# Rinoahu/SwiftOrtho

Measured on AMD Instinct MI355X. Metric: M query-aa/s scanned all-vs-all, higher is better.
Workload: dtype u8/int16/int32 (5-bit packed residues, packed 16-bit score-only DP, int32 traced DP); 1 GPU; BASELINE config 3: 100000 synthetic proteins x 300 aa self-search, seed 11111011111, aa9, -M 120000000, -c 50000 (2 chunks), -e 1e-5, -v 500; query_aa=30007201, rows=1618760

## Files before the change

### swiftortho_amd/csrc/k_ixsort.hip

```cpp
#include "common.h"
#include "kernels.h"

#define IXS_G 512
#define IXS_T1 1024
#define IXS_BINS_MAX 8192
#define IXS_W 16384
#define IXS_T2 512

static inline int ixs_wsh(u32 NC) {
    int wsh = 0;
    while ((((u64)NC + (1ull << wsh) - 1) >> wsh) > IXS_BINS_MAX) ++wsh;
    return wsh;
}
u32 ixsort_bins(u32 NC) { return (u32)(((u64)NC + (1ull << ixs_wsh(NC)) - 1) >> ixs_wsh(NC)); }
size_t ixsort_plan_elems(u32 NC) { return (size_t)ixsort_bins(NC) * IXS_G + 1; }

__device__ __forceinline__ u32 ixs_col() { return (blockIdx.x & 7u) * (IXS_G / 8) + (blockIdx.x >> 3); }
__device__ __forceinline__ void ixs_slice(u32 E, u32& lo, u32& hi) {
    const u64 per = (((u64)E + IXS_G - 1) / IXS_G + 3) & ~3ull;
    lo = (u32)min((u64)E, per * ixs_col()), hi = (u32)min((u64)E, per * (ixs_col() + 1));
}

__global__ __launch_bounds__(IXS_T1) void k_ixs_count(const u32* __restrict__ keys, u32 E, int wsh, u32 nbins, u32* __restrict__ plan ) {
    __shared__ u32 s_cnt[IXS_BINS_MAX];
    for (u32 i = threadIdx.x; i < nbins; i += IXS_T1) s_cnt[i] = 0;
    __syncthreads();
    u32 lo, hi;
    ixs_slice(E, lo, hi);
    for (u32 i = lo + threadIdx.x; i < hi; i += IXS_T1) {
        const u32 k = keys[i];
        if (k != 0xFFFFFFFFu) atomicAdd(&s_cnt[k >> wsh], 1u);
    }
    __syncthreads();
    for (u32 i = threadIdx.x; i < nbins; i += IXS_T1) plan[(size_t)i * IXS_G + ixs_col()] = s_cnt[i];
    if (blockIdx.x == 0 && threadIdx.x == 0) plan[(size_t)nbins * IXS_G] = 0;
}

__global__ __launch_bounds__(IXS_T1) void k_ixs_scatter(const u32* __restrict__ keys, const u64* __restrict__ vals, u32 E, int wsh, u32 nbins,
                                                       const u32* __restrict__ plan , u32* __restrict__ tk, u64* __restrict__ tv) {
    __shared__ u32 s_cur[IXS_BINS_MAX];
    for (u32 i = threadIdx.x; i < nbins; i += IXS_T1) s_cur[i] = plan[(size_t)i * IXS_G + ixs_col()];
    __syncthreads();
    u32 lo, hi;
    ixs_slice(E, lo, hi);
    for (u32 i = lo + threadIdx.x; i < hi; i += IXS_T1) {
        const u32 k = keys[i];
        if (k == 0xFFFFFFFFu) continue;
        const u32 at = atomicAdd(&s_cur[k >> wsh], 1u);
        tk[at] = k, tv[at] = vals[i];
    }
}

__device__ __forceinline__ void ixs_group(const u32* sk, const u64* sv, u32 a, u32 b, u32 idbase, u32* __restrict__ dk,
                                          u64* __restrict__ dv, u32* s_cnt, u32* s_ws) {
    const int tid = threadIdx.x, lane = tid & 63, w = tid >> 6;
    constexpr int PER = IXS_W / IXS_T2;
    for (int i = tid; i < IXS_W; i += IXS_T2) s_cnt[i] = 0;
    __syncthreads();
    for (u32 i = a + (u32)tid; i < b; i += IXS_T2) atomicAdd(&s_cnt[sk[i] - idbase], 1u);
    __syncthreads();
    {
        u32 c[PER], tot = 0;
#pragma unroll
        for (int k = 0; k < PER; ++k) c[k] = s_cnt[tid * PER + k], tot += c[k];
        u32 inc = tot;
#pragma unroll
        for (int o = 1; o < 64; o <<= 1) {
            const u32 x = __shfl_up(inc, o);
            if (lane >= o) inc += x;
        }
        if (lane == 63) s_ws[w] = inc;
        __syncthreads();
        u32 run = a + inc - tot;
        for (int k = 0; k < w; ++k) run += s_ws[k];
#pragma unroll
        for (int k = 0; k < PER; ++k) {
            s_cnt[tid * PER + k] = run;
            run += c[k];
        }
    }
    __syncthreads();
    for (u32 i = a + (u32)tid; i < b; i += IXS_T2) {
        const u32 k = sk[i];
        const u32 at = atomicAdd(&s_cnt[k - idbase], 1u);
        dk[at] = k, dv[at] = sv[i];
    }
    __syncthreads();
}

__global__ __launch_bounds__(IXS_T2) void k_ixs_bin(const u32* __restrict__ tk, const u64* __restrict__ tv, const u32* __restrict__ plan, int wsh,
                                                    u32* ak, u64* av ,
                                                    u32* __restrict__ ok, u64* __restrict__ ov) {
    __shared__ u32 s_cnt[IXS_W];
    __shared__ u32 s_ws[IXS_T2 / 64];
    __shared__ u32 s_sub[34];
    const u32 bin = blockIdx.x;
    const u32 a = plan[(size_t)bin * IXS_G], b = plan[(size_t)(bin + 1) * IXS_G];
    if (a == b) return;
    const u32 idbase = bin << wsh;
    if (wsh <= 14) {
        ixs_group(tk, tv, a, b, idbase, ok, ov, s_cnt, s_ws);
        return;
    }
    const u32 nsub = 1u << (wsh - 14);
    const int tid = threadIdx.x;
    if (tid < 34) s_sub[tid] = 0;
    __syncthreads();
    for (u32 i = a + (u32)tid; i < b; i += IXS_T2) atomicAdd(&s_sub[(tk[i] - idbase) >> 14], 1u);
    __syncthreads();
    if (tid == 0) {
        u32 run = a;
        for (u32 j = 0; j <= nsub; ++j) {
            const u32 c = j < nsub ? s_sub[j] : 0u;
            s_sub[j] = run;
            run += c;
        }
    }
    __syncthreads();
    u32 sub_lo[32];
    for (u32 j = 0; j < nsub; ++j) sub_lo[j] = s_sub[j];
    const u32 sub_end = s_sub[nsub];
    __syncthreads();
    for (u32 i = a + (u32)tid; i < b; i += IXS_T2) {
        const u32 k = tk[i];
        const u32 at = atomicAdd(&s_sub[(k - idbase) >> 14], 1u);
        ak[at] = k, av[at] = tv[i];
    }
    __threadfence();
    __syncthreads();
    for (u32 j = 0; j < nsub; ++j) {
        const u32 sa = sub_lo[j], sb = j + 1 < nsub ? sub_lo[j + 1] : sub_end;
        if (sa < sb) ixs_group(ak, av, sa, sb, idbase + (j << 14), ok, ov, s_cnt, s_ws);
    }
}

const u32* ixsort_count(const u32* kin, u32 n, u32 NC, u32* plan, u32* scan_tmp, hipStream_t st) {
    const int wsh = ixs_wsh(NC);
    const u32 nbins = ixsort_bins(NC);
    hipLaunchKernelGGL(k_ixs_count, dim3(IXS_G), dim3(IXS_T1), 0, st, kin, n, wsh, nbins, plan);
    scan_u32(plan, plan, (size_t)nbins * IXS_G + 1, false, scan_tmp, st);
    return plan + (size_t)nbins * IXS_G;
}
void ixsort_finish(u32* kin, u64* vin, u32 n, u32 NC, const u32* plan, u32* tk, u64* tv, u32* kout, u64* vout, hipStream_t st) {
    if (!n) return;
    const int wsh = ixs_wsh(NC);
    const u32 nbins = ixsort_bins(NC);
    hipLaunchKernelGGL(k_ixs_scatter, dim3(IXS_G), dim3(IXS_T1), 0, st, kin, vin, n, wsh, nbins, plan, tk, tv);
    hipLaunchKernelGGL(k_ixs_bin, dim3(nbins), dim3(IXS_T2), 0, st, tk, tv, plan, wsh, kin, vin, kout, vout);
}
void ixsort_pairs(u32* kin, u64* vin, u32 E, u32 NC, u32* plan, u32* scan_tmp, u32* tk, u64* tv, u32* kout, u64* vout, hipStream_t st) {
    if (!E) return;
    (void)ixsort_count(kin, E, NC, plan, scan_tmp, st);
    ixsort_finish(kin, vin, E, NC, plan, tk, tv, kout, vout, st);
}
```

### swiftortho_amd/csrc/tune.h

```cpp
#pragma once
#include <cstdlib>

#define SOHIT_TUNE_TABLE(X)                                                                                                                                     \
                                                                                                                              \
    X(B, ug1, "SOHIT_UG1", 1, "bucketed passes: singleton groups to k_ungap1 (0: everything to k_ungap)")                                                     \
    X(B, ug1_chain, "SOHIT_UG1_CHAIN", 1, "... and the groups of two and more hits to k_ungap2 (0: to k_ungap, which then skips the singletons)")              \
    X(B, count_steps, "SOHIT_UG_COUNT", 0, "counting instances of the extension kernels: so_counters.ungap_steps, groups_single, groups_chain")                \
    X(B, ungapq, "SOHIT_UNGAPQ", 1, "sparse passes of queries up to 512 residues: hits alone on their diagonal by k_ungapq, a wave per query (0: every hit through the sorted keys)")     \
    X(I, uq_cache, "SOHIT_UQ_CACHE", -1, "... its hit ordinals per query whose index entries stay in registers between the two walks, in steps of 64 (-1: the compiled 1024; 0: every entry read twice; tests move the boundary)") \
    X(I, uq_chains, "SOHIT_UQ_CHAINS", -1, "... what it leaves over sorted per query (k_uqsort_wave: a wave's registers, k_uqsort_wg: a workgroup's LDS) and chained by k_ungap2 from the list of group heads (0: library segmented sort + k_ungap + k_first_touch; N > 0: the largest tier holds N keys -- tests reach the in-place instance with small inputs)") \
    X(B, ug_w32, "SOHIT_UG_W32", 1, "bucketed passes hand k_ungap the buckets' 32-bit words (0: 64-bit keys; no k_ungap1 then)")                               \
                                                                                                             \
    X(B, bucket, "SOHIT_BUCKET", 1, "bucketed diagonal binning (0: every pass on the sorted path)")                                                            \
    X(I, bucket_min, "SOHIT_BUCKET_MIN", 192, "hits per bucket below which a pass takes the sorted path (0: bucketed whenever possible)")                      \
    X(I, bucket_avg, "SOHIT_BUCKET_AVG", 2560, "average bucket size the band-range width is chosen for")                                                       \
    X(I, count_tab, "SOHIT_COUNT_TAB", 1, "bucketed passes: hits per (tile, range) from the range boundaries of the ordered index buckets when a batch brings a chunk two passes and more (0: always the counting pass over the entries; 2: always both, compared -- tests; 3: always)") \
    X(B, bucket_best, "SOHIT_BUCKET_BEST", 1, "best diagonal per subject by the per-bucket reduction (0: sort of the pass records)")                           \
    X(B, bands, "SOHIT_BANDS", 1, "diagonal bands follow the subjects' lengths (0: one band per subject)")                                                     \
    X(B, lk_wide, "SOHIT_LK_WIDE", 0, "8-byte index addends whatever the field widths")                                                                        \
    X(B, qclass, "SOHIT_QCLASS", 1, "queries of a batch in length-class order (0: file order)")                                                                \
    X(B, pass_merge, "SOHIT_PASS_MERGE", 1, "neighbouring length classes that take the sorted path anyway share one pass")                                     \
    X(B, ksc_lazy, "SOHIT_KSC_LAZY", 1, "k-mer orders computed for the queries that reach their frequency cap, when they do (a query below it keeps every window whatever the order; 0: for every query, with the batch)") \
    X(B, bounds_ahead, "SOHIT_BOUNDS_AHEAD", 1, "the next chunk's bucket bounds (k_bounds) on the side stream beside this chunk's seed stage (0: in front of its own)")     \
    X(I, segsort, "SOHIT_SEGSORT", 1, "sorted path: segmented sort of the keys inside each query (0: device-wide sort)")                                        \
    X(I, write_threads, "SOHIT_WRITE_THREADS", 48, "so_write_sc: formatter threads (at most the host's cores)")                                                                          \
                                                                                                                                 \
    X(I, cand_limit, "SOHIT_CAND_LIMIT", 0, "tests: candidate-store size at which a batch is split (0: 2^32 - 16)")                                            \
                                                                                                                                         \
    X(B, align_pk, "SOHIT_ALIGN_PK", 1, "packed 16-bit score-only aligner where the scores fit")                                                               \
    X(B, align_lane, "SOHIT_ALIGN_LANE", 1, "score-only rounds: one lane per alignment pair (k_align_lane) when no sequence reaches 4096 residues (0: k_align_pk)")            \
    X(I, align_lane_min, "SOHIT_ALIGN_LANE_MIN", 1 << 18, "... for rounds of at least this many packed tasks (below: k_align_pk; tests: 0)")                 \
    X(B, align_sort, "SOHIT_ALIGN_SORT", 1, "launch lists ordered by band rows")                                                                               \
    X(I, trace_wave_rows, "SOHIT_TRACE_WAVE_ROWS", 1024, "traceback: bands of this many rows and more are walked by a wave of their own (0: never)")         \
    X(I, trace_wave_max, "SOHIT_TRACE_WAVE_MAX", 32768, "... among the first this many positions of a launch list")                                            \
    X(I, spec, "SOHIT_SPEC", -1, "speculative traces in the first round: 0 off, 1 on, -1 from 2^21 tasks on")                                                  \
    X(D, spec_slack, "SOHIT_SPEC_SLACK", 1e6, "... the guess tests the ungapped score against expect x this (tests: 1e30 = every first-round task traced, 1e-30 = none)")          \
    X(I, spec_cap, "SOHIT_SPEC_CAP", -1, "tests: most speculative traces kept (-1: all)")                                                                      \
    X(I, trace_var_max, "SOHIT_TRACE_VAR_MAX", -1, "tests: trace words a launch list's own-size traces may take, and the fixed-stride slabs' budget (-1: 2^31 / 2^30)") \
    X(I, emit_parts, "SOHIT_EMIT_PARTS", 4, "... and otherwise")                                                                                               \
    X(I, emit_min_rows, "SOHIT_EMIT_MIN_ROWS", 1 << 18, "rows below which the emission is one part")                                                           \
    X(P, test_oom_phase2, "SOHIT_TEST_OOM_PHASE2", 0, "tests: phase 2 of the first batch fails once with an out-of-memory error")                              \
                                                                                                                                 \
    X(I, batch, "SOHIT_BATCH", 0, "queries per device batch (0: 131072, lowered when the candidate estimate asks)")                                            \
    X(I, max_hits, "SOHIT_MAX_HITS", 0, "seed hits per pass (0: 2^30)")                                                                                        \
    X(I, poison, "SOHIT_POISON", -1, "tests: byte every fresh device allocation is filled with (-1: none)")                                                    \
    X(B, hit_cache, "SOHIT_HIT_CACHE", 1, "one released result array is kept for the next search")                                                             \
    X(P, keep_cands, "SOHIT_KEEP_CANDS", 0, "tests: keep every query's candidate list (so_query_candidates)")                                                  \
    X(P, keep_masked, "SOHIT_KEEP_MASKED", 0, "tests: keep the masked queries (so_masked_query)")                                                              \
    X(I, mcl_scratch, "SOHIT_MCL_SCRATCH", -1, "tests: u32 words of expansion / convergence scratch per range of rows (-1: 2^28)")                             \
                                                                                      \
    X(T, orth_tier, "SOHIT_ORTH_TIER", 0, "tests: every run of query rows through one tier of k_orth_run wherever that tier can take it (0 = auto: by run length)") \
                                                                                                  \
    X(T, rbh_tier, "SOHIT_RBH_TIER", 0, "tests: wave = runs of up to 64 rows through k_rbh_run_wave (what auto does), long or sort = every run through the sorted tier (0 = auto: by run length)") \
                                                                                                                                           \
    X(P, exact_threshold, "SOHIT_EXACT_THRESHOLD", 0, "threshold always by the sequential fp64 replay")                                                        \
    X(I, dir_max, "SOHIT_DIR_MAX", -1, "largest -M served by the bitmap + rank directory (-1: 2^31)")                                                          \
                                                                                                                                          \
    X(P, debug, "SOHIT_DEBUG", 0, "per-pass lines on stderr")                                                                                                  \
    X(P, debug_index, "SOHIT_DEBUG_INDEX", 0, "wall laps of the index build on stderr")

#define ORTH_WAVE_ROWS 64
#define ORTH_LDS_ROWS 1024
#define ORTH_LDS_TAXA 512
enum { ORTH_TIER_AUTO = 0, ORTH_TIER_WAVE = 1, ORTH_TIER_LDS = 2, ORTH_TIER_SCRATCH = 3 };
static inline int orth_tier_of(const char* v) {
    switch (v[0]) {
        case 'w': case '1': return ORTH_TIER_WAVE;
        case 'l': case '2': return ORTH_TIER_LDS;
        case 's': case '3': return ORTH_TIER_SCRATCH;
        default: return ORTH_TIER_AUTO;
    }
}

#define RBH_WAVE_ROWS 64

struct Tune {
#define X_B(f, d) bool f = (d) != 0;
#define X_I(f, d) long long f = (d);
#define X_D(f, d) double f = (d);
#define X_P(f, d) bool f = false;
#define X_T(f, d) int f = (d);
#define X(kind, field, env, dflt, text) X_##kind(field, dflt)
    SOHIT_TUNE_TABLE(X)
#undef X
#undef X_B
#undef X_I
#undef X_D
#undef X_P
#undef X_T
    void read() {
#define X_B(f, e) if (const char* v = getenv(e)) f = atoi(v) != 0;
#define X_I(f, e) if (const char* v = getenv(e)) f = strtoll(v, nullptr, 0);
#define X_D(f, e) if (const char* v = getenv(e)) f = atof(v);
#define X_P(f, e) f = getenv(e) != nullptr;
#define X_T(f, e) if (const char* v = getenv(e)) f = orth_tier_of(v);
#define X(kind, field, env, dflt, text) X_##kind(field, env)
        SOHIT_TUNE_TABLE(X)
#undef X
#undef X_B
#undef X_I
#undef X_D
#undef X_P
#undef X_T
    }
};

const Tune& tune();
void set_tune(const Tune* t);
```

Baseline: 699.8 M query-aa/s.

## Restructure index pair sort into two-hop LDS-staged scatter with LDS radix bins

The single-pass scatter into up to 8192 bins is replaced by two hops. The first scatters into at most 128 superbins and the second splits each superbin into its bins. Each hop stages a tile in LDS so global writes land contiguously per destination, instead of spreading atomics over thousands of cursors. Small bins (up to 4096 pairs) are then ordered by a two-pass 7-bit LDS radix sort using wave ballot ranking, and only larger bins keep the per-id counter path. The cost is an extra scan, an extra kernel launch and a full extra read/write pass over the key/value arrays.

```diff
diff --git a/swiftortho_amd/csrc/k_ixsort.hip b/swiftortho_amd/csrc/k_ixsort.hip
--- a/swiftortho_amd/csrc/k_ixsort.hip
+++ b/swiftortho_amd/csrc/k_ixsort.hip
@@ -1,11 +1,17 @@
 #include "common.h"
 #include "kernels.h"
+#include "tune.h"
 
 #define IXS_G 512
 #define IXS_T1 1024
 #define IXS_BINS_MAX 8192
+#define IXS_SB_MAX 128
+#define IXS_K 16
+#define IXS_TH 512
 #define IXS_W 16384
 #define IXS_T2 512
+#define IXS_T3 512
+#define IXS_CAP 4096
 
 static inline int ixs_wsh(u32 NC) {
     int wsh = 0;
@@ -13,7 +19,23 @@
     return wsh;
 }
 u32 ixsort_bins(u32 NC) { return (u32)(((u64)NC + (1ull << ixs_wsh(NC)) - 1) >> ixs_wsh(NC)); }
-size_t ixsort_plan_elems(u32 NC) { return (size_t)ixsort_bins(NC) * IXS_G + 1; }
+static inline int ixs_ssh(u32 nbins) {
+    int ssh = 0;
+    while (((nbins + (1u << ssh) - 1) >> ssh) > IXS_SB_MAX) ++ssh;
+    return ssh;
+}
+static inline u32 ixs_sbins(u32 nbins) { return (nbins + (1u << ixs_ssh(nbins)) - 1) >> ixs_ssh(nbins); }
+static inline size_t ixs_q_at(u32 nbins) { return ((size_t)nbins * IXS_G + 1 + 3) & ~(size_t)3; }
+size_t ixsort_plan_elems(u32 NC) { return ixs_q_at(ixsort_bins(NC)) + (size_t)ixs_sbins(ixsort_bins(NC)) * IXS_G + 1; }
+static inline u32 ixs_k() {
+    const long long k = tune().ixs_k;
+    return k >= 1 && k <= IXS_G / 8 && (k & (k - 1)) == 0 ? (u32)k : (u32)IXS_K;
+}
+
+static inline u32 ixs_cap() {
+    const long long cap = tune().ixs_cap;
+    return cap >= 0 && cap <= IXS_CAP ? (u32)cap : (u32)IXS_CAP;
+}
 
 __device__ __forceinline__ u32 ixs_col() { return (blockIdx.x & 7u) * (IXS_G / 8) + (blockIdx.x >> 3); }
 __device__ __forceinline__ void ixs_slice(u32 E, u32& lo, u32& hi) {
@@ -21,7 +43,8 @@
     lo = (u32)min((u64)E, per * ixs_col()), hi = (u32)min((u64)E, per * (ixs_col() + 1));
 }
 
-__global__ __launch_bounds__(IXS_T1) void k_ixs_count(const u32* __restrict__ keys, u32 E, int wsh, u32 nbins, u32* __restrict__ plan ) {
+__global__ __launch_bounds__(IXS_T1) void k_ixs_count(const u32* __restrict__ keys, u32 E, int wsh, u32 nbins, int ssh, u32 nsb,
+                                                     u32* __restrict__ plan , u32* __restrict__ qplan ) {
     __shared__ u32 s_cnt[IXS_BINS_MAX];
     for (u32 i = threadIdx.x; i < nbins; i += IXS_T1) s_cnt[i] = 0;
     __syncthreads();
@@ -33,22 +56,89 @@
     }
     __syncthreads();
     for (u32 i = threadIdx.x; i < nbins; i += IXS_T1) plan[(size_t)i * IXS_G + ixs_col()] = s_cnt[i];
-    if (blockIdx.x == 0 && threadIdx.x == 0) plan[(size_t)nbins * IXS_G] = 0;
-}
-
-__global__ __launch_bounds__(IXS_T1) void k_ixs_scatter(const u32* __restrict__ keys, const u64* __restrict__ vals, u32 E, int wsh, u32 nbins,
-                                                       const u32* __restrict__ plan , u32* __restrict__ tk, u64* __restrict__ tv) {
-    __shared__ u32 s_cur[IXS_BINS_MAX];
-    for (u32 i = threadIdx.x; i < nbins; i += IXS_T1) s_cur[i] = plan[(size_t)i * IXS_G + ixs_col()];
+    for (u32 s = threadIdx.x; s < nsb; s += IXS_T1) {
+        u32 c = 0;
+        for (u32 b = s << ssh, e = min(nbins, (s + 1) << ssh); b < e; ++b) c += s_cnt[b];
+        qplan[(size_t)s * IXS_G + ixs_col()] = c;
+    }
+    if (blockIdx.x == 0 && threadIdx.x == 0) plan[(size_t)nbins * IXS_G] = 0, qplan[(size_t)nsb * IXS_G] = 0;
+}
+
+template <int T, int IT>
+__device__ __forceinline__ void ixs_hop(const u32* __restrict__ keys, const u64* __restrict__ vals, u32 lo, u32 hi, int sh, u32 dbase, u32 nd, u32* s_cur,
+                                        u32* __restrict__ dk, u64* __restrict__ dv) {
+    __shared__ u32 s_hist[IXS_SB_MAX], s_off[IXS_SB_MAX], s_tot;
+    __shared__ u32 s_k[T * IT];
+    __shared__ u64 s_v[T * IT];
+    const u32 tid = threadIdx.x;
+    for (u32 t0 = lo; t0 < hi; t0 += T * IT) {
+        if (tid < IXS_SB_MAX) s_hist[tid] = 0;
+        __syncthreads();
+        u32 k[IT], r[IT];
+        u64 v[IT] = {};
+#pragma unroll
+        for (int j = 0; j < IT; ++j) {
+            const u32 i = t0 + (u32)j * T + tid;
+            k[j] = i < hi ? keys[i] : 0xFFFFFFFFu;
+            if (k[j] != 0xFFFFFFFFu) v[j] = vals[i];
+        }
+#pragma unroll
+        for (int j = 0; j < IT; ++j)
+            if (k[j] != 0xFFFFFFFFu) r[j] = atomicAdd(&s_hist[(k[j] >> sh) - dbase], 1u);
+        __syncthreads();
+        if (tid < 64) {
+            const u32 c0 = s_hist[2 * tid], c1 = s_hist[2 * tid + 1];
+            u32 inc = c0 + c1;
+#pragma unroll
+            for (int o = 1; o < 64; o <<= 1) {
+                const u32 x = __shfl_up(inc, o);
+                if (tid >= (u32)o) inc += x;
+            }
+            s_off[2 * tid] = inc - c0 - c1, s_off[2 * tid + 1] = inc - c1;
+            if (tid == 63) s_tot = inc;
+        }
+        __syncthreads();
+#pragma unroll
+        for (int j = 0; j < IT; ++j)
+            if (k[j] != 0xFFFFFFFFu) {
+                const u32 p = s_off[(k[j] >> sh) - dbase] + r[j];
+                s_k[p] = k[j], s_v[p] = v[j];
+            }
+        __syncthreads();
+        const u32 n = s_tot;
+        for (u32 p = tid; p < n; p += T) {
+            const u32 kk = s_k[p], d = (kk >> sh) - dbase;
+            const u32 at = s_cur[d] + (p - s_off[d]);
+            dk[at] = kk, dv[at] = s_v[p];
+        }
+        __syncthreads();
+        if (tid < nd) s_cur[tid] += s_hist[tid];
+    }
+}
+
+__global__ __launch_bounds__(IXS_T1) void k_ixs_hop1(const u32* __restrict__ keys, const u64* __restrict__ vals, u32 E, int sh, u32 nsb,
+                                                    const u32* __restrict__ qplan, u32* __restrict__ tk, u64* __restrict__ tv) {
+    __shared__ u32 s_cur[IXS_SB_MAX];
+    if (threadIdx.x < nsb) s_cur[threadIdx.x] = qplan[(size_t)threadIdx.x * IXS_G + ixs_col()];
     __syncthreads();
     u32 lo, hi;
     ixs_slice(E, lo, hi);
-    for (u32 i = lo + threadIdx.x; i < hi; i += IXS_T1) {
-        const u32 k = keys[i];
-        if (k == 0xFFFFFFFFu) continue;
-        const u32 at = atomicAdd(&s_cur[k >> wsh], 1u);
-        tk[at] = k, tv[at] = vals[i];
-    }
+    ixs_hop<IXS_T1, 4>(keys, vals, lo, hi, sh, 0u, nsb, s_cur, tk, tv);
+}
+
+__global__ __launch_bounds__(IXS_TH) void k_ixs_hop2(const u32* __restrict__ tk, const u64* __restrict__ tv, int wsh, u32 nbins, int ssh, u32 K,
+                                                    const u32* __restrict__ plan , const u32* __restrict__ qplan ,
+                                                    u32* __restrict__ ok, u64* __restrict__ ov) {
+    __shared__ u32 s_cur[IXS_SB_MAX];
+    const u32 per = IXS_G / 8 / K;
+    const u32 r = blockIdx.x >> 3;
+    const u32 S = r / per, t = (blockIdx.x & 7u) * per + r % per;
+    const u32 a = qplan[(size_t)S * IXS_G + (size_t)t * K], b = qplan[(size_t)S * IXS_G + (size_t)(t + 1) * K];
+    if (a == b) return;
+    const u32 b0 = S << ssh, nb = min(1u << ssh, nbins - b0);
+    if (threadIdx.x < nb) s_cur[threadIdx.x] = plan[(size_t)(b0 + threadIdx.x) * IXS_G + (size_t)t * K];
+    __syncthreads();
+    ixs_hop<IXS_TH, 8>(tk, tv, a, b, wsh, b0, nb, s_cur, ok, ov);
 }
 
 __device__ __forceinline__ void ixs_group(const u32* sk, const u64* sv, u32 a, u32 b, u32 idbase, u32* __restrict__ dk,
@@ -88,7 +178,70 @@
     __syncthreads();
 }
 
-__global__ __launch_bounds__(IXS_T2) void k_ixs_bin(const u32* __restrict__ tk, const u64* __restrict__ tv, const u32* __restrict__ plan, int wsh,
+__device__ __forceinline__ void ixs_lds_pass(const u32* src, u32* dst, u32 n, int shift, u32* s_cnt , u32* s_ws) {
+    constexpr u32 NW = IXS_T3 / 64;
+    const u32 tid = threadIdx.x, lane = tid & 63u, w = tid >> 6;
+    const u32 per = (n + IXS_T3 - 1) / IXS_T3 * 64u;
+    const u32 lo = min(n, per * w), hi = min(n, per * (w + 1));
+    s_cnt[2 * tid] = 0, s_cnt[2 * tid + 1] = 0;
+    __syncthreads();
+    for (u32 i = lo + lane; i < hi; i += 64) atomicAdd(&s_cnt[((src[i] >> shift) & 127u) * NW + w], 1u);
+    __syncthreads();
+    {
+        const u32 c0 = s_cnt[2 * tid], c1 = s_cnt[2 * tid + 1];
+        u32 inc = c0 + c1;
+#pragma unroll
+        for (int o = 1; o < 64; o <<= 1) {
+            const u32 x = __shfl_up(inc, o);
+            if (lane >= (u32)o) inc += x;
+        }
+        if (lane == 63) s_ws[w] = inc;
+        __syncthreads();
+        u32 run = inc - c0 - c1;
+        for (u32 k = 0; k < w; ++k) run += s_ws[k];
+        s_cnt[2 * tid] = run, s_cnt[2 * tid + 1] = run + c0;
+    }
+    __syncthreads();
+    for (u32 i0 = lo; i0 < hi; i0 += 64) {
+        const u32 i = i0 + lane;
+        const bool live = i < hi;
+        const u32 x = live ? src[i] : 0u, d = (x >> shift) & 127u;
+        unsigned long long peers = __ballot(live);
+#pragma unroll
+        for (int bit = 0; bit < 7; ++bit) {
+            const unsigned long long m = __ballot((d >> bit) & 1u);
+            peers &= ((d >> bit) & 1u) ? m : ~m;
+        }
+        if (live) {
+            const u32 rank = (u32)__popcll(peers & ((1ull << lane) - 1ull)), cnt = (u32)__popcll(peers);
+            const u32 base = s_cnt[d * NW + w];
+            dst[base + rank] = x;
+            if (rank + 1 == cnt) s_cnt[d * NW + w] = base + cnt;
+        }
+    }
+    __syncthreads();
+}
+
+__global__ __launch_bounds__(IXS_T3) void k_ixs_bin_lds(const u32* __restrict__ tk, const u64* __restrict__ tv, const u32* __restrict__ plan, int wsh, u32 cap,
+                                                        u32* __restrict__ ok, u64* __restrict__ ov) {
+    __shared__ u32 s_a[IXS_CAP], s_b[IXS_CAP];
+    __shared__ u32 s_cnt[128 * (IXS_T3 / 64)];
+    __shared__ u32 s_ws[IXS_T3 / 64];
+    const u32 bin = blockIdx.x;
+    const u32 a = plan[(size_t)bin * IXS_G], n = plan[(size_t)(bin + 1) * IXS_G] - a;
+    if (n == 0 || n > cap || wsh > 14) return;
+    const u32 idbase = bin << wsh;
+    for (u32 i = threadIdx.x; i < n; i += IXS_T3) s_a[i] = (tk[a + i] - idbase) | (i << 14);
+    __syncthreads();
+    ixs_lds_pass(s_a, s_b, n, 0, s_cnt, s_ws);
+    ixs_lds_pass(s_b, s_a, n, 7, s_cnt, s_ws);
+    for (u32 p = threadIdx.x; p < n; p += IXS_T3) {
+        const u32 x = s_a[p];
+        ok[a + p] = idbase + (x & 16383u), ov[a + p] = tv[a + (x >> 14)];
+    }
+}
+
+__global__ __launch_bounds__(IXS_T2) void k_ixs_bin(const u32* __restrict__ tk, const u64* __restrict__ tv, const u32* __restrict__ plan, int wsh, u32 cap,
                                                     u32* ak, u64* av ,
                                                     u32* __restrict__ ok, u64* __restrict__ ov) {
     __shared__ u32 s_cnt[IXS_W];
@@ -96,7 +249,7 @@
     __shared__ u32 s_sub[34];
     const u32 bin = blockIdx.x;
     const u32 a = plan[(size_t)bin * IXS_G], b = plan[(size_t)(bin + 1) * IXS_G];
-    if (a == b) return;
+    if (a == b || (wsh <= 14 && b - a <= cap)) return;
     const u32 idbase = bin << wsh;
     if (wsh <= 14) {
         ixs_group(tk, tv, a, b, idbase, ok, ov, s_cnt, s_ws);
@@ -136,17 +289,24 @@
 
 const u32* ixsort_count(const u32* kin, u32 n, u32 NC, u32* plan, u32* scan_tmp, hipStream_t st) {
     const int wsh = ixs_wsh(NC);
-    const u32 nbins = ixsort_bins(NC);
-    hipLaunchKernelGGL(k_ixs_count, dim3(IXS_G), dim3(IXS_T1), 0, st, kin, n, wsh, nbins, plan);
+    const u32 nbins = ixsort_bins(NC), nsb = ixs_sbins(nbins);
+    u32* qplan = plan + ixs_q_at(nbins);
+    hipLaunchKernelGGL(k_ixs_count, dim3(IXS_G), dim3(IXS_T1), 0, st, kin, n, wsh, nbins, ixs_ssh(nbins), nsb, plan, qplan);
     scan_u32(plan, plan, (size_t)nbins * IXS_G + 1, false, scan_tmp, st);
+    scan_u32(qplan, qplan, (size_t)nsb * IXS_G + 1, false, scan_tmp, st);
     return plan + (size_t)nbins * IXS_G;
 }
 void ixsort_finish(u32* kin, u64* vin, u32 n, u32 NC, const u32* plan, u32* tk, u64* tv, u32* kout, u64* vout, hipStream_t st) {
     if (!n) return;
     const int wsh = ixs_wsh(NC);
-    const u32 nbins = ixsort_bins(NC);
-    hipLaunchKernelGGL(k_ixs_scatter, dim3(IXS_G), dim3(IXS_T1), 0, st, kin, vin, n, wsh, nbins, plan, tk, tv);
-    hipLaunchKernelGGL(k_ixs_bin, dim3(nbins), dim3(IXS_T2), 0, st, tk, tv, plan, wsh, kin, vin, kout, vout);
+    const u32 nbins = ixsort_bins(NC), nsb = ixs_sbins(nbins), K = ixs_k();
+    const int ssh = ixs_ssh(nbins);
+    const u32* qplan = plan + ixs_q_at(nbins);
+    hipLaunchKernelGGL(k_ixs_hop1, dim3(IXS_G), dim3(IXS_T1), 0, st, kin, vin, n, wsh + ssh, nsb, qplan, tk, tv);
+    hipLaunchKernelGGL(k_ixs_hop2, dim3(nsb * (IXS_G / K)), dim3(IXS_TH), 0, st, tk, tv, wsh, nbins, ssh, K, plan, qplan, kin, vin);
+    const u32 cap = ixs_cap();
+    if (cap && wsh <= 14) hipLaunchKernelGGL(k_ixs_bin_lds, dim3(nbins), dim3(IXS_T3), 0, st, kin, vin, plan, wsh, cap, kout, vout);
+    hipLaunchKernelGGL(k_ixs_bin, dim3(nbins), dim3(IXS_T2), 0, st, kin, vin, plan, wsh, cap, tk, tv, kout, vout);
 }
 void ixsort_pairs(u32* kin, u64* vin, u32 E, u32 NC, u32* plan, u32* scan_tmp, u32* tk, u64* tv, u32* kout, u64* vout, hipStream_t st) {
     if (!E) return;
diff --git a/swiftortho_amd/csrc/tune.h b/swiftortho_amd/csrc/tune.h
--- a/swiftortho_amd/csrc/tune.h
+++ b/swiftortho_amd/csrc/tune.h
@@ -55,6 +55,8 @@
                                                                                                                                            \
     X(P, exact_threshold, "SOHIT_EXACT_THRESHOLD", 0, "threshold always by the sequential fp64 replay")                                                        \
     X(I, dir_max, "SOHIT_DIR_MAX", -1, "largest -M served by the bitmap + rank directory (-1: 2^31)")                                                          \
+    X(I, ixs_k, "SOHIT_IXS_K", -1, "pair grouping, second hop: slices per workgroup, a power of two up to 64 (-1: the compiled 16)")                            \
+    X(I, ixs_cap, "SOHIT_IXS_CAP", -1, "pair grouping, bins: most pairs of a bin ordered in the LDS, up to 4096 (-1: 4096; 0: every bin by the counters per id; tests move the boundary)") \
                                                                                                                                           \
     X(P, debug, "SOHIT_DEBUG", 0, "per-pass lines on stderr")                                                                                                  \
     X(P, debug_index, "SOHIT_DEBUG_INDEX", 0, "wall laps of the index build on stderr")
```

Result: faster. 712.4 M query-aa/s (median of 6 runs) (+1.8%).
